# chengruiz/cusrl

Measured on AMD Instinct MI355X. Metric: env_steps_per_sec, higher is better.
Workload: dtype f32; 1 GPU; synthetic continuous env 4096x obs48 x act12 per GPU, MLP(256,128) actor-critic, rollout_len=24, ppo preset (5 epochs x 4 minibatches, Adam lr 2e-4); envs_per_gpu=4096, parallelism=dp1, rccl_ranks=0, collectives=none (single process), hipgraph=True, fused_env=True, captured_env_steps=24, epoch_graph_updates=432, unjoined_steps_captured=20, autoreset=False

## Files before the change

cusrl_amd/csrc/gradient.hip:

```cpp
#include "common.hpp"

namespace cusrl {

constexpr int kNormMaxBlocks = 64;
constexpr int kMaxClipPartials = 1 << 16;
constexpr int kNormFloatsPerBlock = 256 * 16;

__global__ __launch_bounds__(kBlock) void sumsq_partials_kernel(const float *__restrict__ g, int64_t n,
                                                                double *__restrict__ partials) {
    __shared__ double scratch[kWavesPerBlock];
    double acc = 0.0;
    const int64_t n4 = n / 4;
    const float4 *__restrict__ g4 = reinterpret_cast<const float4 *>(g);
    for (int64_t i = int64_t(blockIdx.x) * kBlock + threadIdx.x; i < n4; i += int64_t(gridDim.x) * kBlock) {
        const float4 v = g4[i];
        acc += double(v.x * v.x + v.y * v.y) + double(v.z * v.z + v.w * v.w);
    }
    if (blockIdx.x == 0 && threadIdx.x < n - n4 * 4) {
        const float v = g[n4 * 4 + threadIdx.x];
        acc += double(v * v);
    }
    const double total = block_sum(acc, scratch);
    if (threadIdx.x == 0) partials[blockIdx.x] = total;
}
// ... 302 lines not shown
    adam_step_kernel<<<int(blocks > 1024 ? 1024 : blocks), kBlock, 0, as_stream(stream)>>>(
        param, grad, exp_avg, exp_avg_sq, step, lr, num_a > 0 ? clip_partials_a : nullptr, clip_partials_b, int(num_b), norm_out,
        norm_accumulator, step_mirror, ticket, n, a);
    return launch_status();
}

namespace cusrl {

struct GradPiece {
    const float *src;
    int64_t offset, numel, row_stride;
    int32_t splits, wide;
};

struct GradTable {
    int32_t n;
    int32_t block_start[CUSRL_MAX_FIELDS + 1];
    GradPiece piece[CUSRL_MAX_FIELDS];
};

constexpr int kAssemblePerBlock = kBlock * 4;
constexpr int kAssembleWideCols = 16;
constexpr int kAssembleWideSplits = 16;

__global__ __launch_bounds__(kBlock) void assemble_gradients_kernel(const GradTable tab, float *__restrict__ flat,
                                                                    double *__restrict__ sumsq, int sumsq_base) {
    __shared__ double sq_scratch[kWavesPerBlock];
    double sq = 0.0;
    const int blk = blockIdx.x;
    int f = 0;
#pragma unroll
    for (int i = 1; i < CUSRL_MAX_FIELDS; ++i) f += (i < tab.n && blk >= tab.block_start[i]) ? 1 : 0;
    const GradPiece piece = tab.piece[f];
    const float *__restrict__ src = piece.src;
    const int64_t n = piece.numel;
    const int64_t stride = piece.row_stride;
    if (piece.wide) {
        __shared__ float red[kBlock];
        const int c = threadIdx.x % kAssembleWideCols, g = threadIdx.x / kAssembleWideCols;
        constexpr int kGroups = kBlock / kAssembleWideCols;
        const int64_t e = int64_t(blk - tab.block_start[f]) * kAssembleWideCols + c;
        float total = 0.f;
        if (e < n) {
            int s = g;
            for (; s + 3 * kGroups < piece.splits; s += 4 * kGroups) {
                const float a = src[int64_t(s) * stride + e], b = src[int64_t(s + kGroups) * stride + e],
                            c2 = src[int64_t(s + 2 * kGroups) * stride + e], d = src[int64_t(s + 3 * kGroups) * stride + e];
                total += (a + b) + (c2 + d);
            }
            for (; s < piece.splits; s += kGroups) total += src[int64_t(s) * stride + e];
        }
        red[threadIdx.x] = total;
        __syncthreads();
        if (g == 0 && e < n) {
            float sum = red[c];
#pragma unroll
            for (int k = 1; k < kGroups; ++k) sum += red[k * kAssembleWideCols + c];
            flat[piece.offset + e] = sum;
            sq = double(sum * sum);
// ... 9 lines not shown
    for (int k = 0; k < 4; ++k) {
        const int64_t e = base + int64_t(k) * kBlock;
        if (e >= n) break;
        float total = 0.f;
        int s = 0;
        for (; s + 4 <= piece.splits; s += 4) {
            const float a = src[int64_t(s) * stride + e], b = src[int64_t(s + 1) * stride + e],
                        c = src[int64_t(s + 2) * stride + e], d = src[int64_t(s + 3) * stride + e];
            total += (a + b) + (c + d);
        }
        for (; s < piece.splits; ++s) total += src[int64_t(s) * stride + e];
        flat[piece.offset + e] = total;
        sq += double(total * total);
    }
    if (sumsq) {
        const double total_sq = block_sum(sq, sq_scratch);
        if (threadIdx.x == 0) sumsq[sumsq_base + blk] = total_sq;
    }
}

}

static int64_t assemble_blocks(const cusrl_grad_piece_t &p) {
    return cusrl::ceil_div(p.numel, p.splits > cusrl::kAssembleWideSplits ? cusrl::kAssembleWideCols : cusrl::kAssemblePerBlock);
}

extern "C" int64_t cusrl_assemble_gradients_blocks(const cusrl_grad_piece_t *pieces, int64_t num_pieces) {
    if (num_pieces < 0 || (num_pieces > 0 && !pieces)) return -1;
    int64_t blocks = 0;
    for (int64_t i = 0; i < num_pieces; ++i) {
        if (pieces[i].numel < 0 || pieces[i].splits < 0) return -1;
        blocks += assemble_blocks(pieces[i]);
    }
    return blocks;
}

extern "C" int cusrl_assemble_gradients(const cusrl_grad_piece_t *pieces, int64_t num_pieces, float *flat,
                                        double *sumsq_partials, void *stream) {
    using namespace cusrl;
    if (num_pieces < 0 || (num_pieces > 0 && (!pieces || !flat))) return CUSRL_E_INVALID;
    int64_t sumsq_base = 0;
    for (int64_t first = 0; first < num_pieces; first += CUSRL_MAX_FIELDS) {
        GradTable tab;
        tab.n = int32_t(num_pieces - first < CUSRL_MAX_FIELDS ? num_pieces - first : CUSRL_MAX_FIELDS);
        int64_t blocks = 0;
        for (int i = 0; i < tab.n; ++i) {
            const cusrl_grad_piece_t &p = pieces[first + i];
            if (p.numel < 0 || p.offset < 0 || p.splits < 0 || (p.splits > 0 && !p.src)) return CUSRL_E_INVALID;
            const int64_t row_stride = p.row_stride > 0 ? p.row_stride : p.numel;
            if (row_stride < p.numel || p.splits > INT32_MAX) return CUSRL_E_INVALID;
            const bool wide = p.splits > kAssembleWideSplits;
            tab.block_start[i] = int32_t(blocks);
            tab.piece[i] = GradPiece{static_cast<const float *>(p.src), p.offset, p.numel, row_stride, int32_t(p.splits), wide};
            blocks += ceil_div(p.numel, wide ? kAssembleWideCols : kAssemblePerBlock);
            if (blocks > INT32_MAX) return CUSRL_E_UNSUPPORTED;
        }
        tab.block_start[tab.n] = int32_t(blocks);
        if (blocks == 0) continue;
        if (sumsq_base + blocks > kMaxClipPartials && sumsq_partials) return CUSRL_E_UNSUPPORTED;
        assemble_gradients_kernel<<<uint32_t(blocks), kBlock, 0, as_stream(stream)>>>(tab, flat, sumsq_partials, int(sumsq_base));
        if (int rc = launch_status()) return rc;
        sumsq_base += blocks;
    }
    return 0;
}

extern "C" int64_t cusrl_adam_step_normed_workspace_bytes(void) { return int64_t(sizeof(cusrl::NormedWorkspace)); }

extern "C" int cusrl_adam_step_normed(float *param, const float *grad, float *exp_avg, float *exp_avg_sq, float *step,
                                      const float *lr, int64_t n, double beta1, double beta2, double eps, double weight_decay,
                                      int decoupled_weight_decay, int maximize, const float *norm_grad, int64_t norm_n,
                                      void *workspace, float max_norm, float *norm_out, float *norm_accumulator,
                                      float *step_mirror, uint32_t *ticket, void *stream) {
    using namespace cusrl;
    if (n <= 0 || !param || !grad || !exp_avg || !exp_avg_sq || !step || !lr || !ticket) return CUSRL_E_INVALID;
    if (norm_n <= 0 || !norm_grad || !workspace) return CUSRL_E_INVALID;
    if (!aligned(param, 16) || !aligned(grad, 16) || !aligned(exp_avg, 16) || !aligned(exp_avg_sq, 16) ||
// ... 16 lines not shown
```

cusrl_amd/csrc/input_layer.hip:

```cpp
#include "common.hpp"

namespace cusrl {

typedef float mfma_f32x4 __attribute__((ext_vector_type(4)));

constexpr int kInColsPerWave = 64;

__device__ __forceinline__ float4 masked(const float4 &g, const float4 &y) {
    return make_float4(y.x > 0.f ? g.x : 0.f, y.y > 0.f ? g.y : 0.f, y.z > 0.f ? g.z : 0.f, y.w > 0.f ? g.w : 0.f);
}

constexpr int kInWaves = 8;
constexpr int kInThreads = kInWaves * kWave;
constexpr int kInQuads = 4;
constexpr int kInChunk = 4 * kInQuads;

template <bool kMask>
__global__ __launch_bounds__(kInThreads) void input_layer_bwd_kernel(const float *__restrict__ grad, const float *__restrict__ output,
                                                                     const float *__restrict__ input, int64_t rows, int H, int K,
                                                                     int rows_per_block, float *__restrict__ partials,
                                                                     int64_t stride) {
    __shared__ float4 exchange[kInWaves][16][kWave];
    const int lane = threadIdx.x & (kWave - 1), wave = threadIdx.x / kWave;
    const int i = lane & 15, kk = lane >> 4;
// ... 97 lines not shown

static int input_layer_rows_per_block(int64_t rows, int64_t H) {
    const int64_t column_groups = H / kInColsPerWave;
    int64_t row_blocks = ceil_div(256, column_groups);
    if (ceil_div(rows, 512) > row_blocks) row_blocks = ceil_div(rows, 512);
    const int64_t most = ceil_div(rows, kInChunk);
    if (row_blocks > most) row_blocks = most;
    return int(ceil_div(ceil_div(rows, row_blocks), kInChunk) * kInChunk);
}

}

using namespace cusrl;

extern "C" int cusrl_input_layer_supported(int64_t in_features, int64_t out_features) {
    return in_features >= 4 && in_features % 4 == 0 && in_features / 4 <= 15 && out_features >= kInColsPerWave &&
           out_features % kInColsPerWave == 0 && out_features <= 4096;
}

extern "C" int64_t cusrl_input_layer_row_blocks(int64_t rows, int64_t out_features) {
    return rows <= 0 || out_features < kInColsPerWave ? 0 : ceil_div(rows, input_layer_rows_per_block(rows, out_features));
}

extern "C" int cusrl_input_layer_bwd(const float *grad_out, const float *output, const float *input, int64_t rows,
                                     int64_t in_features, int64_t out_features, float *partials, float *grads, void *stream) {
    if (rows <= 0 || !grad_out || !input || !partials || !grads) return CUSRL_E_INVALID;
    if (!cusrl_input_layer_supported(in_features, out_features)) return CUSRL_E_UNSUPPORTED;
    if (!aligned(grad_out, 16) || !aligned(input, 16) || (output && !aligned(output, 16)) || !aligned(partials, 16) ||
        !aligned(grads, 16))
        return CUSRL_E_UNSUPPORTED;
    const int per_block = input_layer_rows_per_block(rows, out_features);
    const int64_t blocks = ceil_div(rows, per_block);
    if (blocks > INT32_MAX) return CUSRL_E_UNSUPPORTED;
    const int64_t width = out_features * in_features + out_features;
    const dim3 grid(uint32_t(blocks), uint32_t(out_features / kInColsPerWave));
    hipStream_t s = as_stream(stream);
    if (output)
        hipLaunchKernelGGL((input_layer_bwd_kernel<true>), grid, dim3(kInThreads), 0, s, grad_out, output, input, rows,
                           int(out_features), int(in_features), per_block, partials, width);
    else
        hipLaunchKernelGGL((input_layer_bwd_kernel<false>), grid, dim3(kInThreads), 0, s, grad_out, output, input, rows,
                           int(out_features), int(in_features), per_block, partials, width);
    if (int rc = launch_status()) return rc;
    hipLaunchKernelGGL(input_layer_sum_rows_kernel, dim3(uint32_t(ceil_div(width / 4, kInReduceCols))), dim3(kBlock), 0, s, partials,
                       int(blocks), width, width, grads);
    return launch_status();
}
```

cusrl_amd/csrc/narrow_linear.hip:

```cpp
#include <stdlib.h>

#include "common.hpp"

namespace cusrl {

static int head_rows_per_block() {
    const int v = int(option(kOptHeadRows));
    return v >= 8 && v <= 4096 ? v : 96;
}
constexpr int head_batch(int O) { return O > 8 ? 2 : 4; }
constexpr int kHeadBiasPad = 16;

template <int O, bool kReluInput>
__global__ __launch_bounds__(kBlock) void narrow_linear_bwd_kernel(const float *__restrict__ grad_out,
                                                                   const float *__restrict__ input,
                                                                   const float *__restrict__ weight,
                                                                   float *__restrict__ grad_input,
                                                                   float *__restrict__ partials, int64_t rows, int K,
                                                                   int rows_per_block) {
    extern __shared__ float4 red[];
    constexpr int SL = O + 1;
    const int lpr = K / 4;
    const int groups = kBlock / lpr;
    const int col = threadIdx.x % lpr, sub = threadIdx.x / lpr;
// ... 125 lines not shown
    const int64_t row0 = wave * (kRowsPerWave * kInFlight);
    if (row0 >= rows) return;
    const float b = bias ? bias[0] : 0.f;
    float acc[kInFlight] = {0.f, 0.f, 0.f, 0.f};
    for (int c = sub; c < chunks; c += kLanes) {
        const float4 w = reinterpret_cast<const float4 *>(weight)[c];
        float4 x[kInFlight];
#pragma unroll
        for (int k = 0; k < kInFlight; ++k) {
            const int64_t row = min(row0 + int64_t(k) * kRowsPerWave + rloc, rows - 1);
            x[k] = reinterpret_cast<const float4 *>(input)[row * chunks + c];
        }
#pragma unroll
        for (int k = 0; k < kInFlight; ++k)
            acc[k] += (x[k].x * w.x + x[k].y * w.y) + (x[k].z * w.z + x[k].w * w.w);
    }
#pragma unroll
    for (int k = 0; k < kInFlight; ++k) {
        float v = acc[k];
#pragma unroll
        for (int off = kLanes / 2; off > 0; off >>= 1) v += __shfl_xor(v, off, kWave);
        const int64_t row = row0 + int64_t(k) * kRowsPerWave + rloc;
        if (sub == 0 && row < rows) output[row] = v + b;
    }
}

static bool narrow_shape_ok(int64_t K, int64_t O) {
    if (O < 1 || O > 16 || K < 32 || K > 1024 || K % 4) return false;
    const int64_t lpr = K / 4;
    return (lpr & (lpr - 1)) == 0;
}

template <int O, bool kReluInput>
static int launch_narrow_bwd_as(const float *grad_out, const float *input, const float *weight, float *grad_input,
                                float *partials, int64_t rows, int K, int64_t blocks, hipStream_t s) {
    const int lpr = K / 4, groups = kBlock / lpr;
    const size_t lds = size_t(groups) * (O + 1) * lpr * sizeof(float4) + size_t(groups) * kHeadBiasPad * sizeof(float);
    if (lds > 64 * 1024) {
        hipError_t err = hipFuncSetAttribute(reinterpret_cast<const void *>(&narrow_linear_bwd_kernel<O, kReluInput>),
                                             hipFuncAttributeMaxDynamicSharedMemorySize, int(lds));
        if (err != hipSuccess) return int(err);
    }
    hipLaunchKernelGGL((narrow_linear_bwd_kernel<O, kReluInput>), dim3(uint32_t(blocks)), dim3(kBlock), lds, s, grad_out,
                       input, weight, grad_input, partials, rows, K, head_rows_per_block());
    return launch_status();
}
// ... 28 lines not shown
    hipStream_t s = as_stream(stream);
    const int K = int(in_features);
    const int64_t blocks = ceil_div(rows, int64_t(head_rows_per_block()));
    const bool relu = relu_input != 0;
    int rc = 0;
    switch (out_features) {
#define CUSRL_NARROW_CASE(N) \
    case N: rc = launch_narrow_bwd<N>(grad_out, input, weight, grad_input, partials, rows, K, blocks, relu, s); break;
        CUSRL_NARROW_CASE(1) CUSRL_NARROW_CASE(2) CUSRL_NARROW_CASE(3) CUSRL_NARROW_CASE(4)
        CUSRL_NARROW_CASE(5) CUSRL_NARROW_CASE(6) CUSRL_NARROW_CASE(7) CUSRL_NARROW_CASE(8)
        CUSRL_NARROW_CASE(9) CUSRL_NARROW_CASE(10) CUSRL_NARROW_CASE(11) CUSRL_NARROW_CASE(12)
        CUSRL_NARROW_CASE(13) CUSRL_NARROW_CASE(14) CUSRL_NARROW_CASE(15) CUSRL_NARROW_CASE(16)
#undef CUSRL_NARROW_CASE
        default: return CUSRL_E_UNSUPPORTED;
    }
    if (rc) return rc;
    if (!packed) return 0;
    const int H = (int(out_features) + 1) * K + kHeadBiasPad;
    hipLaunchKernelGGL(narrow_linear_finalize_kernel, dim3(uint32_t(ceil_div(H, 64))), dim3(kBlock), 0, s, partials,
                       blocks, H, packed);
    return launch_status();
}

extern "C" int cusrl_narrow_linear_fwd(const float *input, const float *weight, const float *bias, float *output,
                                       int64_t rows, int64_t in_features, int64_t out_features, void *stream) {
    using namespace cusrl;
    if (!input || !weight || !output || rows <= 0) return CUSRL_E_INVALID;
    if (out_features != 1 || !narrow_shape_ok(in_features, 1)) return CUSRL_E_UNSUPPORTED;
    if (!aligned(input, 16) || !aligned(weight, 16)) return CUSRL_E_UNSUPPORTED;
    const int K = int(in_features), lanes = K / 4 >= kWave ? kWave : K / 4;
    const int64_t waves = ceil_div(rows, int64_t(kWave / lanes) * 4), blocks = ceil_div(waves, int64_t(kWavesPerBlock));
    if (blocks > INT32_MAX) return CUSRL_E_UNSUPPORTED;
    hipStream_t s = as_stream(stream);
    switch (lanes) {
#define CUSRL_DOT_CASE(N)                                                                                              \
    case N:                                                                                                            \
        hipLaunchKernelGGL(narrow_dot_fwd_kernel<N>, dim3(uint32_t(blocks)), dim3(kBlock), 0, s, input, weight, bias,   \
                           output, rows, K);                                                                           \
        break;
        CUSRL_DOT_CASE(8) CUSRL_DOT_CASE(16) CUSRL_DOT_CASE(32) CUSRL_DOT_CASE(64)
#undef CUSRL_DOT_CASE
        default: return CUSRL_E_UNSUPPORTED;
    }
    return launch_status();
}
```

cusrl_amd/nn/module.py:

```python

from __future__ import annotations

from collections.abc import Iterable, Sequence
from contextlib import contextmanager
from dataclasses import dataclass
from typing import Any

import torch
from torch import nn
from torch.nn.functional import linear

from cusrl_amd.utils import switches
from cusrl_amd.utils.nest import iterate_nested

__all__ = ["Linear", "LinearFp32", "fused_inference_layers", "linear_act", "Mlp", "Module", "ModuleFactory", "disable_autocast",
           "double_differentiable", "is_unit_gradient", "register_unit_gradient", "resolve_activation_fn"]


def disable_autocast(device_type: str):
    return torch.autocast(device_type=device_type, enabled=False)


_split_grad_sink: dict[int, torch.Tensor] | None = None


_plain_linear_depth = 0
_WIDE_MIN_ROWS = switches.read("WIDE_LINEAR_MIN_ROWS")
_INPUT_LAYER_KERNEL = switches.read("INPUT_LAYER_KERNEL")


_unit_gradients: dict[int, "weakref.ref[torch.Tensor]"] = {}


def register_unit_gradient(ones: torch.Tensor) -> torch.Tensor:
    import weakref

    address = ones.data_ptr()
    _unit_gradients[address] = weakref.ref(ones)
    weakref.finalize(ones, _forget_unit_gradient, address)
    return ones


def _forget_unit_gradient(address: int) -> None:
    ref = _unit_gradients.get(address)
    if ref is not None and ref() is None:
        del _unit_gradients[address]


def is_unit_gradient(grad: torch.Tensor | None) -> bool:
    if grad is None or grad.dim() != 0:
        return False
    ref = _unit_gradients.get(grad.data_ptr())
    return ref is not None and ref() is not None


@contextmanager
def double_differentiable():
    global _plain_linear_depth
    _plain_linear_depth += 1
    try:
        yield
    finally:
        _plain_linear_depth -= 1


@contextmanager
def collect_split_weight_grads():
    global _split_grad_sink
    previous, _split_grad_sink = _split_grad_sink, {}
    try:
        yield _split_grad_sink
    finally:
        _split_grad_sink = previous


def _hand_over(sink, key, gradient):
    from cusrl_amd import ops

    if not isinstance(gradient, ops.DeferredColumns):
        return gradient
    if sink is not None and key is not None and key not in sink:
        sink[key] = gradient
        return None
    return gradient.materialize()


class _WideBatchLinear(torch.autograd.Function):

    @staticmethod
    def forward(ctx, input, weight, bias, splits, relu):
        if relu:
            output = torch._addmm_activation(bias, input, weight.t())
# ... 2 lines not shown
        else:
            output = _one_output_linear(input, weight, bias)
            ctx.save_for_backward(input, weight)
        ctx.splits, ctx.relu, ctx.has_bias = splits, relu, bias is not None
        ctx.bias_key = bias.data_ptr() if bias is not None else None
        ctx.narrow = ((not relu) and input.is_contiguous() and weight.is_contiguous() and input.data_ptr() % 16 == 0
                      and _narrow_head(weight))
        ctx.input_is_relu_output = getattr(input, "_cusrl_relu_output", False)
        return output

    @staticmethod
    @torch.autograd.function.once_differentiable
    def backward(ctx, grad_output):
        from cusrl_amd import ops

        if ctx.relu:
            input, weight, output = ctx.saved_tensors
            sink = _split_grad_sink
            premasked = getattr(grad_output, "_cusrl_premasked", None)
            if (_INPUT_LAYER_KERNEL and premasked is None and not ctx.needs_input_grad[0] and ctx.needs_input_grad[1]
                    and ctx.has_bias and ctx.needs_input_grad[2]):
                grad_output = grad_output.contiguous()
                if ops.input_layer_supported(grad_output, output, input, weight):
                    d_weight, d_bias = ops.input_layer_backward(grad_output, output, input)
                    return None, d_weight, d_bias, None, None
            if premasked is not None and premasked[1] == grad_output._version and ctx.has_bias:
                grad_bias = premasked[0]
            else:
                grad_output, grad_bias = ops.relu_backward_bias(
                    grad_output.contiguous(), output, defer=sink is not None and ctx.has_bias and ctx.needs_input_grad[2])
            grad_bias = _hand_over(sink, ctx.bias_key, grad_bias)
        else:
            input, weight = ctx.saved_tensors
            if ctx.narrow and ctx.needs_input_grad[1]:
                fuse_relu = ctx.input_is_relu_output and ctx.needs_input_grad[0]
                sink = _split_grad_sink
                grad_input, grad_weight, grad_bias, masked_colsum = ops.narrow_linear_backward(
                    grad_output.contiguous(), input, weight, need_input_grad=ctx.needs_input_grad[0], relu_input=fuse_relu,
                    defer=sink is not None)
                grad_weight = _hand_over(sink, weight.data_ptr(), grad_weight)
                grad_bias = _hand_over(sink, ctx.bias_key, grad_bias) if ctx.has_bias else None
                if fuse_relu:
                    grad_input._cusrl_premasked = (masked_colsum, grad_input._version)
                return grad_input, grad_weight, (grad_bias if ctx.has_bias else None), None, None
            grad_bias = None
            if ctx.has_bias and ctx.needs_input_grad[2]:
                _, grad_bias = ops.relu_backward_bias(grad_output.contiguous(), None)
        grad_input = grad_weight = None
        if ctx.needs_input_grad[0]:
            grad_input = grad_output @ weight
        if ctx.needs_input_grad[1]:
            rows, splits = input.shape[0], ctx.splits
            if splits > 1:
                gy = grad_output.reshape(splits, rows // splits, -1)
                slabs = torch.bmm(gy.transpose(1, 2), input.reshape(splits, rows // splits, -1))
                sink = _split_grad_sink
                if sink is not None and weight.data_ptr() not in sink:
                    sink[weight.data_ptr()] = slabs
                else:
                    grad_weight = ops.sum_slabs(slabs)
            else:
                grad_weight = grad_output.t() @ input
        return grad_input, grad_weight, grad_bias, None, None


def _one_output_linear(input: torch.Tensor, weight: torch.Tensor, bias: torch.Tensor | None) -> torch.Tensor:
    from cusrl_amd import ops

    if weight.shape[0] == 1 and ops.narrow_linear_forward_supported(input, weight):
        return ops.narrow_linear_forward(input, weight, bias)
    return linear(input, weight, bias)


def _narrow_head(weight: torch.Tensor) -> bool:
    from cusrl_amd import ops

    return (weight.shape[0] <= 16 and weight.data_ptr() % 16 == 0
            and ops.narrow_linear_supported(weight.shape[1], weight.shape[0]))


def _batch_splits(rows: int) -> int:
    if rows < 4096:
        return 1
    splits = 1
    while splits < 32 and rows % (splits * 2) == 0 and rows // (splits * 2) >= 1024:
        splits *= 2
    return splits


def _device_fp32(input: torch.Tensor, weight: torch.Tensor) -> bool:
    return (input.dim() == 2 and input.is_cuda and input.dtype == torch.float32 and weight.dtype == torch.float32
            and not torch.is_autocast_enabled("cuda"))

# ... 185 lines not shown
```

cusrl_amd/ops/__init__.py:

```python

from __future__ import annotations

import os
from collections.abc import Sequence

import torch

from cusrl_amd import _native
from cusrl_amd._native import Field, MirrorField, PackedField, check
from cusrl_amd.ops._common import (
    LaunchObserver, _checked, _f32, _flag, _modified_in_place, _observed, _ptr, _raw_stream, _row_bytes, _stream, require_device,
    set_launch_observer,
)
from cusrl_amd.ops.advantage import (
    adv_stats_finalize, col_stats, gae, merge_mean_var, next_value, normalize_, normalize_from_gathered_, normalize_from_partials_,
    packed_mean_var,
)
from cusrl_amd.ops.auxiliary import (
    accumulate_scalars_, amp_prepare, amp_prepare_supported, amp_style_reward_, amp_style_reward_mean_, bce_pair_fwd_bwd,
    column_mse_fwd_bwd, column_table, masked_col_stats, mse_loss_fwd_bwd, resolve_columns, reward_shaping_, rms_merge_,
    rms_normalize, rnd_reward_, sumsq_fwd_bwd,
)
from cusrl_amd.ops.buffer import (
    HostCounter, RecordPack, _row_elems, assign_rows, buffer_push, compact_flags, gather_rows, gather_rows_packed, make_push_table,
    push_table, scatter_rows, splice_rows, window_indices,
)
from cusrl_amd.ops.gradient import (
    DeferredColumns, adam_norm_workspace, adam_step, adam_step_normed, adam_step_window, assemble_gradients, clip_grad_norm_,
    grad_sumsq, sum_slabs,
)
from cusrl_amd.ops.graph import graph_census, graph_replace_memsets
from cusrl_amd.ops.loss import (
    LOSS_DEFER, DeferredLoss, _optional_rows, categorical_policy_stats, categorical_terms_bwd, categorical_terms_fwd, policy_stats,
    policy_terms_bwd, policy_terms_fwd, ppo_loss_accepts_std_vector, ppo_loss_categorical_fwd_bwd, ppo_loss_fwd_bwd,
    value_loss_fwd_bwd,
)
from cusrl_amd.ops.mlp import (
    _HEAD_PAD, input_layer_backward, input_layer_supported, mlp2_forward, mlp2_forward_supported, narrow_linear_backward,
    narrow_linear_forward, narrow_linear_forward_supported, narrow_linear_supported, relu_backward_bias,
)
from cusrl_amd.ops.recurrent import (
    gru_bias_partial_rows, gru_bias_partials_supported, gru_gates_backward, gru_gates_forward, lstm_gates_backward,
    lstm_gates_forward, rnn_cell_backward, rnn_cell_forward,
)
from cusrl_amd.ops.rollout import (
    PendingStepEpilogue, categorical_sample_logp, episode_stats, normal_sample_logp, step_epilogue, synthetic_env_step,
)
from cusrl_amd.ops.symmetry import (
    _mirror_table, _rows_2d, mirror_mse_fwd_bwd, mirror_rows, mirror_rows_bwd, symmetrize_mean_var_,
)
```

cusrl_amd/ops/mlp.py:

```python

from __future__ import annotations

import torch

from cusrl_amd import _native
from cusrl_amd.ops._common import _checked, _f32, _observed, _ptr, _stream
from cusrl_amd.ops.gradient import DeferredColumns


def relu_backward_bias(grad_output: torch.Tensor, output: torch.Tensor | None, defer: bool = False):
    grad_output = _f32(grad_output, "grad_output")
    H = grad_output.shape[-1]
    rows = grad_output.numel() // H
    lib = _native.lib()
    num_partials = max(int(lib.cusrl_colsum_num_partials(rows, H)), 1)
    partials = torch.empty((num_partials, H), dtype=torch.float32, device=grad_output.device)
    chunkable = H % 4 == 0 and H // 4 <= 256 and 256 % (H // 4) == 0
    defer = defer and chunkable and grad_output.data_ptr() % 16 == 0 and (output is None or output.data_ptr() % 16 == 0)
    colsum = None if defer else torch.empty(H, dtype=torch.float32, device=grad_output.device)
    if output is None:
        grad_in, out_ptr, in_ptr = grad_output, None, None
    else:
        output = _f32(output, "output")
        grad_in = torch.empty_like(grad_output)
        out_ptr, in_ptr = output.data_ptr(), grad_in.data_ptr()
    _checked.cusrl_relu_bwd_colsum(grad_output.data_ptr(), out_ptr, in_ptr, partials.data_ptr(), _ptr(colsum), rows, H, _stream())
    return grad_in, (DeferredColumns(partials, num_partials, H, 0, H) if colsum is None else colsum)


def input_layer_supported(grad_output: torch.Tensor, output: torch.Tensor | None, input: torch.Tensor, weight: torch.Tensor) -> bool:
    H, K = weight.shape
    tensors = [grad_output, input] + ([] if output is None else [output])
    return (bool(_native.lib().cusrl_input_layer_supported(K, H)) and input.dim() == 2 and grad_output.shape == (input.shape[0], H)
            and all(t.is_cuda and t.dtype == torch.float32 and t.is_contiguous() and t.data_ptr() % 16 == 0 for t in tensors)
            and (output is None or output.shape == grad_output.shape) and input.shape[0] > 0)


def input_layer_backward(grad_output: torch.Tensor, output: torch.Tensor | None, input: torch.Tensor) -> tuple[torch.Tensor, torch.Tensor]:
    grad_output, input = _f32(grad_output, "grad_output"), _f32(input, "input")
    rows, K = input.shape
    H = grad_output.shape[-1]
    lib = _native.lib()
    dev = input.device
    width = H * K + H
    partials = torch.empty((int(lib.cusrl_input_layer_row_blocks(rows, H)), width), dtype=torch.float32, device=dev)
    grads = torch.empty(width, dtype=torch.float32, device=dev)
    _observed("cusrl_input_layer_bwd", grad_output.data_ptr(), _ptr(None if output is None else _f32(output, "output")),
            input.data_ptr(), rows, K, H, partials.data_ptr(), grads.data_ptr(),
            nbytes=lambda: rows * 4 * ((2 if output is not None else 1) * H + K) + (partials.numel() * 2 + width) * 4)
    return grads[: H * K].view(H, K), grads[H * K :]


_HEAD_PAD = 16


def narrow_linear_supported(in_features: int, out_features: int) -> bool:
    return bool(_native.lib().cusrl_narrow_linear_supported(in_features, out_features))


def narrow_linear_forward_supported(input: torch.Tensor, weight: torch.Tensor) -> bool:
    return (weight.dim() == 2 and weight.shape[0] == 1 and input.dim() == 2 and input.is_cuda and input.dtype == torch.float32
            and weight.dtype == torch.float32 and input.is_contiguous() and weight.is_contiguous() and input.shape[0] > 0
            and input.data_ptr() % 16 == 0 and weight.data_ptr() % 16 == 0 and narrow_linear_supported(weight.shape[1], 1))


def narrow_linear_forward(input: torch.Tensor, weight: torch.Tensor, bias: torch.Tensor | None) -> torch.Tensor:
    input, weight = _f32(input, "input"), _f32(weight, "weight")
    rows, K = input.shape
    out = torch.empty((rows, 1), dtype=torch.float32, device=input.device)
    _checked.cusrl_narrow_linear_fwd(input.data_ptr(), weight.data_ptr(), _ptr(None if bias is None else _f32(bias, "bias")),
            out.data_ptr(), rows, K, 1, _stream())
    return out


def mlp2_forward_supported(input: torch.Tensor, layers) -> bool:
    w1, b1, w2, b2, w3, b3 = layers
    tensors = [input, w1, b1, w2, b2, w3] + ([b3] if b3 is not None else [])
    if input.dim() != 2 or input.shape[0] == 0 or any(
            (not t.is_cuda) or t.dtype != torch.float32 or (not t.is_contiguous()) or t.data_ptr() % 16 for t in tensors):
        return False
    if w1.dim() != 2 or w2.dim() != 2 or w3.dim() != 2 or w1.shape[1] != input.shape[1] or w2.shape[1] != w1.shape[0] \
            or w3.shape[1] != w2.shape[0] or b1.numel() != w1.shape[0] or b2.numel() != w2.shape[0] \
            or (b3 is not None and b3.numel() != w3.shape[0]):
        return False
    return bool(_native.lib().cusrl_mlp2_forward_supported(w1.shape[1], w1.shape[0], w2.shape[0], w3.shape[0]))


def mlp2_forward(input: torch.Tensor, layers, std: torch.Tensor | None = None, eps: torch.Tensor | None = None,
                 repeat_std: bool = True):
    w1, b1, w2, b2, w3, b3 = layers
    input = _f32(input, "input")
    rows, K = input.shape
    out_features = w3.shape[0]
    out = torch.empty((rows, out_features), dtype=torch.float32, device=input.device)
# ... 40 lines not shown
```

cusrl_amd/template/actor_critic.py:

```python

from __future__ import annotations

from collections.abc import Callable, Iterable, Mapping, Sequence
from contextlib import contextmanager
from dataclasses import dataclass
from typing import Any

import torch

from cusrl_amd.nn.actor import Actor, Value
from cusrl_amd.nn.module import collect_split_weight_grads, register_unit_gradient
from cusrl_amd.template.agent import Agent, AgentFactory, preserve_io_format
from cusrl_amd.template.buffer import Buffer, Sampler
from cusrl_amd.template.environment import EnvironmentSpec
from cusrl_amd.template.hook import Hook, HookComposite
from cusrl_amd.template.optimizer import OptimizerFactory, build_optimizer
from cusrl_amd.utils import switches
from cusrl_amd.utils.config import CONFIG
from cusrl_amd.utils.distributed import FlatGradients, UnjoinedStep, broadcast_parameters, reduce_gradients

__all__ = ["ActorCritic", "ActorCriticFactory", "HookList", "StepContext", "StepPlan", "plan_step"]


def _hashable(value):
# ... 395 lines not shown
                yield dict(metadata), drawn.permutations[epoch, lo:hi]

    def _zero_grad(self):
        if self.flat_optimizer is not None:
            self.flat_optimizer.discard_pending_clip()
        if self.flat_gradients is None:
            self.optimizer.zero_grad()
        elif not self.flat_gradients.intact():
            self.flat_gradients.attach()

    def _backward(self, loss):
        flat = self.flat_gradients
        roots = list(loss) if isinstance(loss, (list, tuple)) else [loss]
        if len(roots) > 1:
            roots = [t for t in roots if isinstance(t, torch.Tensor) and t.requires_grad] or roots[:1]
        if flat is None:
            total = roots[0]
            for term in roots[1:]:
                total = total + term
            self.grad_scaler.scale(total).backward()
            return

        def differentiate(roots, units, ids, retain=False):
            with collect_split_weight_grads() as slabs:
                grads = torch.autograd.grad(roots, [flat.params[i] for i in ids], grad_outputs=units, allow_unused=True,
                                            retain_graph=retain)
            return grads, slabs

        units = [self._unit_gradient(term) for term in roots]
        plan = self.step_plan()
        branch_root = getattr(loss, "branch", None)
        if branch_root is not None and (plan.mode == ONE_PASS or len(roots) != len(loss)):
            torch.cuda.current_stream().wait_stream(branch_root[1])
            branch_root = None
        if branch_root is None and plan.mode != SPLIT:
            flat.assemble(*differentiate(roots, units, range(len(flat.params))))
            return
        from cusrl_amd.utils import distributed
        from cusrl_amd.utils.config import configure_distributed

        main, branch, context = torch.cuda.current_stream(), self._branch_stream, self.step_context
        split = plan.mode == SPLIT
        unjoined = plan.mode == UNJOINED and context.unjoined is not None
        multi_rank = configure_distributed()
        want_sumsq = unjoined and not multi_rank
        critic_roots, critic_units, other_roots, other_units = roots, units, roots, units
        if branch_root is not None:
# ... 123 lines not shown
```

include/cusrl_hip.h:

```cpp
#ifndef CUSRL_HIP_H
#define CUSRL_HIP_H

#include <stdint.h>

#ifdef __cplusplus
extern "C" {
#endif

#define CUSRL_ABI_VERSION 7
#define CUSRL_MAX_FIELDS 24
#define CUSRL_MAX_PACKED 16
#define CUSRL_MAX_RECORD_BYTES 1024
#define CUSRL_MAX_MIRROR_FIELDS 24
#define CUSRL_MAX_SYMMETRIZE_CHANNELS 4096

#define CUSRL_E_INVALID (-1)
#define CUSRL_E_TOO_MANY (-2)
#define CUSRL_E_UNSUPPORTED (-3)
#define CUSRL_E_COMM (-4)

typedef struct {
    const void *src;
    void *dst;
    int64_t row_bytes;
// ... 142 lines not shown
                                   double *partials, float *out, void *stream);

int cusrl_policy_terms_fwd(const float *mean, const float *std, int64_t std_rows, const float *action,
                           const float *old_logp, int64_t B, int64_t A, float *logp_out, float *entropy_out,
                           float *logp_ratio_out, float *ratio_out, void *stream);
int cusrl_policy_terms_bwd(const float *mean, const float *std, int64_t std_rows, const float *action, const float *ratio,
                           const float *g_logp, const float *g_entropy, const float *g_logp_ratio, const float *g_ratio,
                           int64_t B, int64_t A, float *d_mean, float *d_std, float *d_std_partials, void *stream);
int64_t cusrl_policy_terms_std_partial_rows(int64_t B);
int cusrl_categorical_terms_fwd(const float *logits, const float *action, const float *old_logp, int64_t B, int64_t A,
                                float *logp_out, float *entropy_out, float *logp_ratio_out, float *ratio_out, void *stream);
int cusrl_categorical_terms_bwd(const float *logits, const float *action, const float *ratio, const float *g_logp,
                                const float *g_entropy, const float *g_logp_ratio, const float *g_ratio, int64_t B,
                                int64_t A, float *d_logits, void *stream);

int cusrl_relu_bwd_colsum(const float *grad, const float *output, float *grad_in, float *partials, float *colsum,
                          int64_t rows, int64_t H, void *stream);
int64_t cusrl_colsum_num_partials(int64_t rows, int64_t H);

int cusrl_input_layer_bwd(const float *grad_out, const float *output, const float *input, int64_t rows, int64_t in_features,
                          int64_t out_features, float *partials, float *grads, void *stream);
int cusrl_input_layer_supported(int64_t in_features, int64_t out_features);
int64_t cusrl_input_layer_row_blocks(int64_t rows, int64_t out_features);

int cusrl_narrow_linear_bwd(const float *grad_out, const float *input, const float *weight, float *grad_input,
                            float *partials, float *packed, int64_t rows, int64_t in_features, int64_t out_features,
                            int relu_input, void *stream);
int64_t cusrl_narrow_linear_num_partials(int64_t rows);
int cusrl_narrow_linear_supported(int64_t in_features, int64_t out_features);
int cusrl_narrow_linear_fwd(const float *input, const float *weight, const float *bias, float *output, int64_t rows,
                            int64_t in_features, int64_t out_features, void *stream);

int cusrl_mlp2_forward(const float *input, int64_t rows, int64_t in_features, const float *w1, const float *b1, int64_t hidden1,
                       const float *w2, const float *b2, int64_t hidden2, const float *w3, const float *b3, int64_t out_features,
                       float *output, const float *std, const float *eps, float *action, float *logp, float *std_out,
                       void *stream);
int cusrl_mlp2_forward_supported(int64_t in_features, int64_t hidden1, int64_t hidden2, int64_t out_features);

int cusrl_clip_grad_norm(float *grad, int64_t n, float max_norm, double *partials, float *norm_out, void *stream);
int64_t cusrl_clip_grad_norm_num_partials(int64_t n);

typedef struct {
    const void *src;
    int64_t offset;
    int64_t numel;
    int64_t splits;
    int64_t row_stride;
} cusrl_grad_piece_t;
int cusrl_assemble_gradients(const cusrl_grad_piece_t *pieces, int64_t num_pieces, float *flat, double *sumsq_partials,
                             void *stream);
int64_t cusrl_assemble_gradients_blocks(const cusrl_grad_piece_t *pieces, int64_t num_pieces);

int cusrl_grad_sumsq(const float *grad, int64_t n, double *partials, void *stream);

// ... 113 lines not shown
```

Before: 20.93 million env-steps/s.

## Vectorize wide gradient assembly, defer input-layer row reduction, add narrow head forward

```diff
diff --git a/cusrl_amd/csrc/gradient.hip b/cusrl_amd/csrc/gradient.hip
--- a/cusrl_amd/csrc/gradient.hip
+++ b/cusrl_amd/csrc/gradient.hip
@@ -348,6 +348,15 @@
 constexpr int kAssemblePerBlock = kBlock * 4;
 constexpr int kAssembleWideCols = 16;
 constexpr int kAssembleWideSplits = 16;
+constexpr int kAssembleWideVecCols = 4 * kAssembleWideCols;
+
+static int wide_kind(const void *src, int64_t offset, int64_t numel, int64_t row_stride, int64_t splits) {
+    if (splits <= kAssembleWideSplits) return 0;
+    return aligned(src, 16) && row_stride % 4 == 0 && offset % 4 == 0 && numel % 4 == 0 ? 2 : 1;
+}
+static int64_t wide_block_elements(int kind) {
+    return kind == 2 ? kAssembleWideVecCols : (kind == 1 ? kAssembleWideCols : kAssemblePerBlock);
+}
 
 __global__ __launch_bounds__(kBlock) void assemble_gradients_kernel(const GradTable tab, float *__restrict__ flat,
                                                                     double *__restrict__ sumsq, int sumsq_base) {
@@ -361,6 +370,47 @@
     const float *__restrict__ src = piece.src;
     const int64_t n = piece.numel;
     const int64_t stride = piece.row_stride;
+    if (piece.wide == 2) {
+        __shared__ float4 red4[kBlock];
+        const int c = threadIdx.x % kAssembleWideCols, g = threadIdx.x / kAssembleWideCols;
+        constexpr int kGroups = kBlock / kAssembleWideCols;
+        const int64_t e = int64_t(blk - tab.block_start[f]) * kAssembleWideVecCols + 4 * c;
+        float4 total = make_float4(0.f, 0.f, 0.f, 0.f);
+        if (e < n) {
+            const float4 *__restrict__ base = reinterpret_cast<const float4 *>(src + e);
+            const int64_t stride4 = stride / 4;
+            int s = g;
+            for (; s + 3 * kGroups < piece.splits; s += 4 * kGroups) {
+                const float4 a = base[int64_t(s) * stride4], b = base[int64_t(s + kGroups) * stride4],
+                             c2 = base[int64_t(s + 2 * kGroups) * stride4], d = base[int64_t(s + 3 * kGroups) * stride4];
+                total.x += (a.x + b.x) + (c2.x + d.x), total.y += (a.y + b.y) + (c2.y + d.y);
+                total.z += (a.z + b.z) + (c2.z + d.z), total.w += (a.w + b.w) + (c2.w + d.w);
+            }
+            for (; s < piece.splits; s += kGroups) {
+                const float4 a = base[int64_t(s) * stride4];
+                total.x += a.x, total.y += a.y, total.z += a.z, total.w += a.w;
+            }
+        }
+        red4[threadIdx.x] = total;
+        __syncthreads();
+        if (g == 0 && e < n) {
+            float4 sum = red4[c];
+#pragma unroll
+            for (int k = 1; k < kGroups; ++k) {
+                const float4 v = red4[k * kAssembleWideCols + c];
+                sum.x += v.x, sum.y += v.y, sum.z += v.z, sum.w += v.w;
+            }
+            float *out = flat + piece.offset + e;
+            if (aligned_ptr16(out)) *reinterpret_cast<float4 *>(out) = sum;
+            else out[0] = sum.x, out[1] = sum.y, out[2] = sum.z, out[3] = sum.w;
+            sq = (double(sum.x * sum.x) + double(sum.y * sum.y)) + (double(sum.z * sum.z) + double(sum.w * sum.w));
+        }
+        if (sumsq) {
+            const double total_sq = block_sum(sq, sq_scratch);
+            if (threadIdx.x == 0) sumsq[sumsq_base + blk] = total_sq;
+        }
+        return;
+    }
     if (piece.wide) {
         __shared__ float red[kBlock];
         const int c = threadIdx.x % kAssembleWideCols, g = threadIdx.x / kAssembleWideCols;
@@ -416,7 +466,8 @@
 }
 
 static int64_t assemble_blocks(const cusrl_grad_piece_t &p) {
-    return cusrl::ceil_div(p.numel, p.splits > cusrl::kAssembleWideSplits ? cusrl::kAssembleWideCols : cusrl::kAssemblePerBlock);
+    const int64_t row_stride = p.row_stride > 0 ? p.row_stride : p.numel;
+    return cusrl::ceil_div(p.numel, cusrl::wide_block_elements(cusrl::wide_kind(p.src, p.offset, p.numel, row_stride, p.splits)));
 }
 
 extern "C" int64_t cusrl_assemble_gradients_blocks(const cusrl_grad_piece_t *pieces, int64_t num_pieces) {
@@ -443,10 +494,10 @@
             if (p.numel < 0 || p.offset < 0 || p.splits < 0 || (p.splits > 0 && !p.src)) return CUSRL_E_INVALID;
             const int64_t row_stride = p.row_stride > 0 ? p.row_stride : p.numel;
             if (row_stride < p.numel || p.splits > INT32_MAX) return CUSRL_E_INVALID;
-            const bool wide = p.splits > kAssembleWideSplits;
+            const int wide = wide_kind(p.src, p.offset, p.numel, row_stride, p.splits);
             tab.block_start[i] = int32_t(blocks);
             tab.piece[i] = GradPiece{static_cast<const float *>(p.src), p.offset, p.numel, row_stride, int32_t(p.splits), wide};
-            blocks += ceil_div(p.numel, wide ? kAssembleWideCols : kAssemblePerBlock);
+            blocks += ceil_div(p.numel, wide_block_elements(wide));
             if (blocks > INT32_MAX) return CUSRL_E_UNSUPPORTED;
         }
         tab.block_start[tab.n] = int32_t(blocks);
diff --git a/cusrl_amd/csrc/input_layer.hip b/cusrl_amd/csrc/input_layer.hip
--- a/cusrl_amd/csrc/input_layer.hip
+++ b/cusrl_amd/csrc/input_layer.hip
@@ -143,27 +143,42 @@
     return rows <= 0 || out_features < kInColsPerWave ? 0 : ceil_div(rows, input_layer_rows_per_block(rows, out_features));
 }
 
-extern "C" int cusrl_input_layer_bwd(const float *grad_out, const float *output, const float *input, int64_t rows,
-                                     int64_t in_features, int64_t out_features, float *partials, float *grads, void *stream) {
-    if (rows <= 0 || !grad_out || !input || !partials || !grads) return CUSRL_E_INVALID;
+static int launch_input_layer_pass(const float *grad_out, const float *output, const float *input, int64_t rows, int64_t in_features,
+                                   int64_t out_features, float *partials, int64_t *row_blocks, hipStream_t s) {
     if (!cusrl_input_layer_supported(in_features, out_features)) return CUSRL_E_UNSUPPORTED;
-    if (!aligned(grad_out, 16) || !aligned(input, 16) || (output && !aligned(output, 16)) || !aligned(partials, 16) ||
-        !aligned(grads, 16))
+    if (!aligned(grad_out, 16) || !aligned(input, 16) || (output && !aligned(output, 16)) || !aligned(partials, 16))
         return CUSRL_E_UNSUPPORTED;
     const int per_block = input_layer_rows_per_block(rows, out_features);
     const int64_t blocks = ceil_div(rows, per_block);
     if (blocks > INT32_MAX) return CUSRL_E_UNSUPPORTED;
     const int64_t width = out_features * in_features + out_features;
     const dim3 grid(uint32_t(blocks), uint32_t(out_features / kInColsPerWave));
-    hipStream_t s = as_stream(stream);
     if (output)
         hipLaunchKernelGGL((input_layer_bwd_kernel<true>), grid, dim3(kInThreads), 0, s, grad_out, output, input, rows,
                            int(out_features), int(in_features), per_block, partials, width);
     else
         hipLaunchKernelGGL((input_layer_bwd_kernel<false>), grid, dim3(kInThreads), 0, s, grad_out, output, input, rows,
                            int(out_features), int(in_features), per_block, partials, width);
-    if (int rc = launch_status()) return rc;
+    *row_blocks = blocks;
+    return launch_status();
+}
+
+extern "C" int cusrl_input_layer_bwd(const float *grad_out, const float *output, const float *input, int64_t rows,
+                                     int64_t in_features, int64_t out_features, float *partials, float *grads, void *stream) {
+    if (rows <= 0 || !grad_out || !input || !partials || !grads) return CUSRL_E_INVALID;
+    if (cusrl_input_layer_supported(in_features, out_features) && !aligned(grads, 16)) return CUSRL_E_UNSUPPORTED;
+    hipStream_t s = as_stream(stream);
+    int64_t blocks = 0;
+    if (int rc = launch_input_layer_pass(grad_out, output, input, rows, in_features, out_features, partials, &blocks, s)) return rc;
+    const int64_t width = out_features * in_features + out_features;
     hipLaunchKernelGGL(input_layer_sum_rows_kernel, dim3(uint32_t(ceil_div(width / 4, kInReduceCols))), dim3(kBlock), 0, s, partials,
                        int(blocks), width, width, grads);
     return launch_status();
 }
+
+extern "C" int cusrl_input_layer_bwd_partials(const float *grad_out, const float *output, const float *input, int64_t rows,
+                                              int64_t in_features, int64_t out_features, float *partials, void *stream) {
+    if (rows <= 0 || !grad_out || !input || !partials) return CUSRL_E_INVALID;
+    int64_t blocks = 0;
+    return launch_input_layer_pass(grad_out, output, input, rows, in_features, out_features, partials, &blocks, as_stream(stream));
+}
diff --git a/cusrl_amd/csrc/narrow_linear.hip b/cusrl_amd/csrc/narrow_linear.hip
--- a/cusrl_amd/csrc/narrow_linear.hip
+++ b/cusrl_amd/csrc/narrow_linear.hip
@@ -171,6 +171,122 @@
         for (int off = kLanes / 2; off > 0; off >>= 1) v += __shfl_xor(v, off, kWave);
         const int64_t row = row0 + int64_t(k) * kRowsPerWave + rloc;
         if (sub == 0 && row < rows) output[row] = v + b;
+    }
+}
+
+constexpr int kHeadFwdInFlight = 4;
+
+template <int N, int kOff>
+__device__ __forceinline__ void head_fwd_halve(float *v, int sub) {
+    const bool hi = (sub & kOff) != 0;
+#pragma unroll
+    for (int i = 0; i < N / 2; ++i) {
+        const float keep = hi ? v[N / 2 + i] : v[i], send = hi ? v[i] : v[N / 2 + i];
+        v[i] = keep + __shfl_xor(send, kOff, kWave);
+    }
+}
+
+template <int NP, int kLanes, bool kRegW>
+__global__ __launch_bounds__(kBlock) void narrow_head_fwd_kernel(const float *__restrict__ input, const float *__restrict__ weight,
+                                                                 const float *__restrict__ bias, float *__restrict__ output,
+                                                                 int64_t rows, int K, int O, int rows_per_block, int vector_store) {
+    extern __shared__ float4 w_lds[];
+    constexpr int kRowsPerWave = kWave / kLanes, kBatch = kRowsPerWave * kHeadFwdInFlight;
+    constexpr int kGroups = NP <= 4 ? 1 : (NP <= 8 ? 2 : 4);
+    const int chunks = K / 4;
+    for (int i = threadIdx.x; i < O * chunks; i += kBlock) w_lds[i] = reinterpret_cast<const float4 *>(weight)[i];
+    __syncthreads();
+    const int lane = threadIdx.x & (kWave - 1), wave = threadIdx.x / kWave;
+    const int sub = lane % kLanes, rloc = lane / kLanes;
+    float4 w[kRegW ? NP : 1];
+    if constexpr (kRegW) {
+#pragma unroll
+        for (int o = 0; o < NP; ++o) {
+            w[o] = make_float4(0.f, 0.f, 0.f, 0.f);
+            if (o < O) w[o] = w_lds[o * chunks + sub];
+        }
+    }
+    const int group = sub / (kLanes / kGroups);
+    const bool holder = sub % (kLanes / kGroups) == 0 && group * 4 < O;
+    const bool biased = holder && bias != nullptr;
+    const float b0 = biased ? bias[group * 4] : 0.f, b1 = biased && group * 4 + 1 < O ? bias[group * 4 + 1] : 0.f;
+    const float b2 = biased && group * 4 + 2 < O ? bias[group * 4 + 2] : 0.f, b3 = biased && group * 4 + 3 < O ? bias[group * 4 + 3] : 0.f;
+    const int64_t row0 = int64_t(blockIdx.x) * rows_per_block;
+    const int64_t row_end = min(row0 + rows_per_block, rows);
+    for (int64_t base = row0 + int64_t(wave) * kBatch; base < row_end; base += int64_t(kWavesPerBlock) * kBatch) {
+        float acc[kHeadFwdInFlight][4 * kGroups];
+#pragma unroll
+        for (int k = 0; k < kHeadFwdInFlight; ++k)
+#pragma unroll
+            for (int o = 0; o < 4 * kGroups; ++o) acc[k][o] = 0.f;
+        for (int c = sub; c < chunks; c += kLanes) {
+            float4 x[kHeadFwdInFlight];
+#pragma unroll
+            for (int k = 0; k < kHeadFwdInFlight; ++k) {
+                const int64_t row = min(base + int64_t(k) * kRowsPerWave + rloc, row_end - 1);
+                x[k] = reinterpret_cast<const float4 *>(input)[row * chunks + c];
+            }
+#pragma unroll
+            for (int o = 0; o < NP; ++o) {
+                float4 wo = make_float4(0.f, 0.f, 0.f, 0.f);
+                if constexpr (kRegW) wo = w[o];
+                else if (o < O) wo = w_lds[o * chunks + c];
+#pragma unroll
+                for (int k = 0; k < kHeadFwdInFlight; ++k)
+                    acc[k][o] = fmaf(x[k].w, wo.w, fmaf(x[k].z, wo.z, fmaf(x[k].y, wo.y, fmaf(x[k].x, wo.x, acc[k][o]))));
+            }
+        }
+#pragma unroll
+        for (int k = 0; k < kHeadFwdInFlight; ++k) {
+            float *v = acc[k];
+            if constexpr (kGroups == 4) head_fwd_halve<16, kLanes / 2>(v, sub), head_fwd_halve<8, kLanes / 4>(v, sub);
+            if constexpr (kGroups == 2) head_fwd_halve<8, kLanes / 2>(v, sub);
+#pragma unroll
+            for (int off = kLanes / (2 * kGroups); off > 0; off >>= 1)
+#pragma unroll
+                for (int i = 0; i < 4; ++i) v[i] += __shfl_xor(v[i], off, kWave);
+            const int64_t row = base + int64_t(k) * kRowsPerWave + rloc;
+            if (holder && row < row_end) {
+                float *out = output + row * O + group * 4;
+                const float4 y = make_float4(v[0] + b0, v[1] + b1, v[2] + b2, v[3] + b3);
+                if (vector_store) {
+                    *reinterpret_cast<float4 *>(out) = y;
+                } else {
+                    out[0] = y.x;
+                    if (group * 4 + 1 < O) out[1] = y.y;
+                    if (group * 4 + 2 < O) out[2] = y.z;
+                    if (group * 4 + 3 < O) out[3] = y.w;
+                }
+            }
+        }
+    }
+}
+
+template <int NP, int kLanes, bool kRegW>
+static int launch_head_fwd_as(const float *input, const float *weight, const float *bias, float *output, int64_t rows, int K,
+                              int O, hipStream_t s) {
+    constexpr int64_t kBlockBatch = int64_t(kWavesPerBlock) * (kWave / kLanes) * kHeadFwdInFlight;
+    const int64_t per_block = ceil_div(ceil_div(rows, 512), kBlockBatch) * kBlockBatch;
+    const int64_t blocks = ceil_div(rows, per_block);
+    if (blocks > INT32_MAX || per_block > INT32_MAX) return CUSRL_E_UNSUPPORTED;
+    const size_t lds = size_t(O) * K * sizeof(float);
+    const int vector_store = O % 4 == 0 && aligned(output, 16) ? 1 : 0;
+    hipLaunchKernelGGL((narrow_head_fwd_kernel<NP, kLanes, kRegW>), dim3(uint32_t(blocks)), dim3(kBlock), lds, s, input, weight,
+                       bias, output, rows, K, O, int(per_block), vector_store);
+    return launch_status();
+}
+
+template <int NP>
+static int launch_head_fwd(const float *input, const float *weight, const float *bias, float *output, int64_t rows, int K, int O,
+                           hipStream_t s) {
+    switch (K / 4) {
+        case 8: return launch_head_fwd_as<NP, 8, true>(input, weight, bias, output, rows, K, O, s);
+        case 16: return launch_head_fwd_as<NP, 16, true>(input, weight, bias, output, rows, K, O, s);
+        case 32: return launch_head_fwd_as<NP, 32, true>(input, weight, bias, output, rows, K, O, s);
+        case 64: return launch_head_fwd_as<NP, 64, true>(input, weight, bias, output, rows, K, O, s);
+        case 128:
+        case 256: return launch_head_fwd_as<NP, 64, false>(input, weight, bias, output, rows, K, O, s);
+        default: return CUSRL_E_UNSUPPORTED;
     }
 }
 
@@ -245,6 +361,27 @@
     return launch_status();
 }
 
+extern "C" int cusrl_narrow_head_fwd_supported(int64_t in_features, int64_t out_features) {
+    return cusrl::narrow_shape_ok(in_features, out_features) ? 1 : 0;
+}
+
+extern "C" int cusrl_narrow_head_fwd(const float *input, const float *weight, const float *bias, float *output, int64_t rows,
+                                     int64_t in_features, int64_t out_features, void *stream) {
+    using namespace cusrl;
+    if (!input || !weight || !output || rows <= 0) return CUSRL_E_INVALID;
+    if (!narrow_shape_ok(in_features, out_features)) return CUSRL_E_UNSUPPORTED;
+    if (!aligned(input, 16) || !aligned(weight, 16) || !aligned(output, 4) || (bias && !aligned(bias, 4))) return CUSRL_E_UNSUPPORTED;
+    hipStream_t s = as_stream(stream);
+    const int K = int(in_features), O = int(out_features);
+    switch ((O + 3) / 4) {
+        case 1: return launch_head_fwd<4>(input, weight, bias, output, rows, K, O, s);
+        case 2: return launch_head_fwd<8>(input, weight, bias, output, rows, K, O, s);
+        case 3: return launch_head_fwd<12>(input, weight, bias, output, rows, K, O, s);
+        case 4: return launch_head_fwd<16>(input, weight, bias, output, rows, K, O, s);
+        default: return CUSRL_E_UNSUPPORTED;
+    }
+}
+
 extern "C" int cusrl_narrow_linear_fwd(const float *input, const float *weight, const float *bias, float *output,
                                        int64_t rows, int64_t in_features, int64_t out_features, void *stream) {
     using namespace cusrl;
diff --git a/cusrl_amd/nn/module.py b/cusrl_amd/nn/module.py
--- a/cusrl_amd/nn/module.py
+++ b/cusrl_amd/nn/module.py
@@ -27,6 +27,8 @@
 _plain_linear_depth = 0
 _WIDE_MIN_ROWS = switches.read("WIDE_LINEAR_MIN_ROWS")
 _INPUT_LAYER_KERNEL = switches.read("INPUT_LAYER_KERNEL")
+_DEFER_INPUT_LAYER_ROWS = True
+_NARROW_HEAD_FORWARD = True
 
 
 _unit_gradients: dict[int, "weakref.ref[torch.Tensor]"] = {}
@@ -64,10 +66,16 @@
         _plain_linear_depth -= 1
 
 
+class _GradSink(dict):
+
+    bottom_rows = False
+
+
 @contextmanager
-def collect_split_weight_grads():
+def collect_split_weight_grads(bottom_rows: bool = False):
     global _split_grad_sink
-    previous, _split_grad_sink = _split_grad_sink, {}
+    previous, _split_grad_sink = _split_grad_sink, _GradSink()
+    _split_grad_sink.bottom_rows = bottom_rows
     try:
         yield _split_grad_sink
     finally:
@@ -116,8 +124,9 @@
                     and ctx.has_bias and ctx.needs_input_grad[2]):
                 grad_output = grad_output.contiguous()
                 if ops.input_layer_supported(grad_output, output, input, weight):
-                    d_weight, d_bias = ops.input_layer_backward(grad_output, output, input)
-                    return None, d_weight, d_bias, None, None
+                    d_weight, d_bias = ops.input_layer_backward(grad_output, output, input,
+                                                                defer=_DEFER_INPUT_LAYER_ROWS and sink is not None and sink.bottom_rows)
+                    return None, _hand_over(sink, weight.data_ptr(), d_weight), _hand_over(sink, ctx.bias_key, d_bias), None, None
             if premasked is not None and premasked[1] == grad_output._version and ctx.has_bias:
                 grad_bias = premasked[0]
             else:
@@ -163,6 +172,9 @@
 
     if weight.shape[0] == 1 and ops.narrow_linear_forward_supported(input, weight):
         return ops.narrow_linear_forward(input, weight, bias)
+    if (_NARROW_HEAD_FORWARD and 2 <= weight.shape[0] <= 16 and ops.narrow_head_forward_supported(input, weight)
+            and (bias is None or (bias.is_cuda and bias.dtype == torch.float32))):
+        return ops.narrow_head_forward(input, weight, bias)
     return linear(input, weight, bias)
 
 
diff --git a/cusrl_amd/ops/__init__.py b/cusrl_amd/ops/__init__.py
--- a/cusrl_amd/ops/__init__.py
+++ b/cusrl_amd/ops/__init__.py
@@ -36,8 +36,8 @@
     value_loss_fwd_bwd,
 )
 from cusrl_amd.ops.mlp import (
-    _HEAD_PAD, input_layer_backward, input_layer_supported, mlp2_forward, mlp2_forward_supported, narrow_linear_backward,
-    narrow_linear_forward, narrow_linear_forward_supported, narrow_linear_supported, relu_backward_bias,
+    _HEAD_PAD, input_layer_backward, input_layer_supported, mlp2_forward, mlp2_forward_supported, narrow_head_forward,
+    narrow_head_forward_supported, narrow_linear_backward, narrow_linear_forward, narrow_linear_forward_supported, narrow_linear_supported, relu_backward_bias,
 )
 from cusrl_amd.ops.recurrent import (
     gru_bias_partial_rows, gru_bias_partials_supported, gru_gates_backward, gru_gates_forward, lstm_gates_backward,
diff --git a/cusrl_amd/ops/mlp.py b/cusrl_amd/ops/mlp.py
--- a/cusrl_amd/ops/mlp.py
+++ b/cusrl_amd/ops/mlp.py
@@ -36,14 +36,20 @@
             and (output is None or output.shape == grad_output.shape) and input.shape[0] > 0)
 
 
-def input_layer_backward(grad_output: torch.Tensor, output: torch.Tensor | None, input: torch.Tensor) -> tuple[torch.Tensor, torch.Tensor]:
+def input_layer_backward(grad_output: torch.Tensor, output: torch.Tensor | None, input: torch.Tensor, defer: bool = False):
     grad_output, input = _f32(grad_output, "grad_output"), _f32(input, "input")
     rows, K = input.shape
     H = grad_output.shape[-1]
     lib = _native.lib()
     dev = input.device
     width = H * K + H
-    partials = torch.empty((int(lib.cusrl_input_layer_row_blocks(rows, H)), width), dtype=torch.float32, device=dev)
+    row_blocks = int(lib.cusrl_input_layer_row_blocks(rows, H))
+    partials = torch.empty((row_blocks, width), dtype=torch.float32, device=dev)
+    if defer:
+        _observed("cusrl_input_layer_bwd_partials", grad_output.data_ptr(), _ptr(None if output is None else _f32(output, "output")),
+                input.data_ptr(), rows, K, H, partials.data_ptr(),
+                nbytes=lambda: rows * 4 * ((2 if output is not None else 1) * H + K) + partials.numel() * 4)
+        return DeferredColumns(partials, row_blocks, width, 0, H * K), DeferredColumns(partials, row_blocks, width, H * K, H)
     grads = torch.empty(width, dtype=torch.float32, device=dev)
     _observed("cusrl_input_layer_bwd", grad_output.data_ptr(), _ptr(None if output is None else _f32(output, "output")),
             input.data_ptr(), rows, K, H, partials.data_ptr(), grads.data_ptr(),
@@ -70,6 +76,23 @@
     out = torch.empty((rows, 1), dtype=torch.float32, device=input.device)
     _checked.cusrl_narrow_linear_fwd(input.data_ptr(), weight.data_ptr(), _ptr(None if bias is None else _f32(bias, "bias")),
             out.data_ptr(), rows, K, 1, _stream())
+    return out
+
+
+def narrow_head_forward_supported(input: torch.Tensor, weight: torch.Tensor) -> bool:
+    return (weight.dim() == 2 and input.dim() == 2 and input.is_cuda and weight.is_cuda and input.dtype == torch.float32
+            and weight.dtype == torch.float32 and input.is_contiguous() and weight.is_contiguous() and input.shape[0] > 0
+            and input.shape[1] == weight.shape[1] and input.data_ptr() % 16 == 0 and weight.data_ptr() % 16 == 0
+            and bool(_native.lib().cusrl_narrow_head_fwd_supported(weight.shape[1], weight.shape[0])))
+
+
+def narrow_head_forward(input: torch.Tensor, weight: torch.Tensor, bias: torch.Tensor | None) -> torch.Tensor:
+    input, weight = _f32(input, "input"), _f32(weight, "weight")
+    rows, K = input.shape
+    O = weight.shape[0]
+    out = torch.empty((rows, O), dtype=torch.float32, device=input.device)
+    _observed("cusrl_narrow_head_fwd", input.data_ptr(), weight.data_ptr(), _ptr(None if bias is None else _f32(bias, "bias")),
+            out.data_ptr(), rows, K, O, nbytes=lambda: 4 * (rows * (K + O) + O * (K + 1)))
     return out
 
 
diff --git a/cusrl_amd/template/actor_critic.py b/cusrl_amd/template/actor_critic.py
--- a/cusrl_amd/template/actor_critic.py
+++ b/cusrl_amd/template/actor_critic.py
@@ -441,7 +441,7 @@
             return
 
         def differentiate(roots, units, ids, retain=False):
-            with collect_split_weight_grads() as slabs:
+            with collect_split_weight_grads(bottom_rows=True) as slabs:
                 grads = torch.autograd.grad(roots, [flat.params[i] for i in ids], grad_outputs=units, allow_unused=True,
                                             retain_graph=retain)
             return grads, slabs
diff --git a/include/cusrl_hip.h b/include/cusrl_hip.h
--- a/include/cusrl_hip.h
+++ b/include/cusrl_hip.h
@@ -188,6 +188,8 @@
                           int64_t out_features, float *partials, float *grads, void *stream);
 int cusrl_input_layer_supported(int64_t in_features, int64_t out_features);
 int64_t cusrl_input_layer_row_blocks(int64_t rows, int64_t out_features);
+int cusrl_input_layer_bwd_partials(const float *grad_out, const float *output, const float *input, int64_t rows,
+                                   int64_t in_features, int64_t out_features, float *partials, void *stream);
 
 int cusrl_narrow_linear_bwd(const float *grad_out, const float *input, const float *weight, float *grad_input,
                             float *partials, float *packed, int64_t rows, int64_t in_features, int64_t out_features,
@@ -196,6 +198,9 @@
 int cusrl_narrow_linear_supported(int64_t in_features, int64_t out_features);
 int cusrl_narrow_linear_fwd(const float *input, const float *weight, const float *bias, float *output, int64_t rows,
                             int64_t in_features, int64_t out_features, void *stream);
+int cusrl_narrow_head_fwd(const float *input, const float *weight, const float *bias, float *output, int64_t rows,
+                          int64_t in_features, int64_t out_features, void *stream);
+int cusrl_narrow_head_fwd_supported(int64_t in_features, int64_t out_features);
 
 int cusrl_mlp2_forward(const float *input, int64_t rows, int64_t in_features, const float *w1, const float *b1, int64_t hidden1,
                        const float *w2, const float *b2, int64_t hidden2, const float *w3, const float *b3, int64_t out_features,
```

Result: no change. 20.75 million env-steps/s (-0.9%).
